# PaddlePaddle/MetaGym

Measured on AMD Instinct MI355X. Metric: env-steps/sec (whole node) at 2^16 parallel envs; 1/2/4/8-GPU scaling, higher is better.
Workload: dtype f32/f64 mixed (reference choreography)

## Files before the change

metagym_amd/csrc/quadrotor.hip:

```cpp
#include <cstdlib>

#include "mg_common.h"
#include "mg_philox.h"

namespace {

#ifndef MG_QUAD_BLOCK
#define MG_QUAD_BLOCK 256
#endif
constexpr int BLOCK = MG_QUAD_BLOCK;
constexpr int WAVES_PER_BLOCK = BLOCK / mg::WAVE;
constexpr int OBS_DIM = 16;

struct QuadK {
    float phi32, phi_over_ra32, inv_jm32, mm32, prec32, ct0_32, ct1_32;
    float quality32, dt32, zoff32, healthy32, fail_range_sq32;
    float lm[4];
    float pc[12];
    float iinv[9];
    float df[9], dm[9];
    float cog[3];
    double prec, half_dt2, half_dt, ct2, quality, inv_quality;
    double min_v, max_v, fail_velocity, fail_w, healthy, xoff, yoff;
    int quality_recip_exact;
    int times, nt, task;
    int auto_reset;
    float init_v_base[3], init_w_base[3];
    double init_v_noisy, init_w_noisy;
    uint64_t seed, env_id_base;
    const int32_t *map;
    int map_h, map_w;
    const float *vtargets;
    int obs_dim;
};

struct Lane {
    float p[3];
    double v[3];
    double w[3];
    float pw[4];
    float R[9];
    double Rd[9];
    float Ri[9];
    double nv, nw;
    float power;
};


__device__ __forceinline__ double dot_row_f32f64(const float *row, const double *x) {
    return fma((double)row[2], x[2], fma((double)row[0], x[0], (double)row[1] * x[1]));
}

__device__ __forceinline__ void mv_f32f64(const float *M, const double *x, double *y) {
#pragma unroll
    for (int r = 0; r < 3; ++r) y[r] = dot_row_f32f64(&M[3 * r], x);
}

__device__ __forceinline__ void mv_f32(const float *M, const float *x, float *y) {
#pragma unroll
    for (int r = 0; r < 2; ++r) y[r] = (M[3 * r] * x[0] + M[3 * r + 1] * x[1]) + M[3 * r + 2] * x[2];
    y[2] = fmaf(M[8], x[2], fmaf(M[6], x[0], M[7] * x[1]));
}

__device__ __forceinline__ void mm_f32(const float *A, const float *B, float *C) {
#pragma unroll
    for (int r = 0; r < 3; ++r)
#pragma unroll
        for (int c = 0; c < 3; ++c)
            C[3 * r + c] = fmaf(A[3 * r + 2], B[6 + c], fmaf(A[3 * r + 1], B[3 + c], A[3 * r] * B[c]));
}

__device__ __forceinline__ void cross_f32(const float *a, const float *b, float *c) {
    float t0 = a[1] * b[2], t1 = a[2] * b[1];
    float t2 = a[2] * b[0], t3 = a[0] * b[2];
    float t4 = a[0] * b[1], t5 = a[1] * b[0];
    c[0] = t0 - t1;
    c[1] = t2 - t3;
    c[2] = t4 - t5;
}

__device__ __forceinline__ double norm3(const double *x) {
    return sqrt(fma(x[2], x[2], fma(x[1], x[1], x[0] * x[0])));
}
__device__ __forceinline__ float sumsq3(const float *x) {
    const float p0 = x[0] * x[0], p1 = x[1] * x[1], p2 = x[2] * x[2];
    return (float)(((double)p0 + (double)p1) + (double)p2);
}

__device__ __forceinline__ void inv3(const float *Af, float *Ainv, double *A) {
#pragma unroll
    for (int i = 0; i < 9; ++i) A[i] = (double)Af[i];
    const double c00 = fma(A[4], A[8], -(A[5] * A[7]));
    const double c01 = fma(A[5], A[6], -(A[3] * A[8]));
    const double c02 = fma(A[3], A[7], -(A[4] * A[6]));
    const double det = fma(A[2], c02, fma(A[1], c01, A[0] * c00));
    const double r = 1.0 / det;
    Ainv[0] = (float)(c00 * r);
    Ainv[3] = (float)(c01 * r);
    Ainv[6] = (float)(c02 * r);
    Ainv[1] = (float)(fma(A[2], A[7], -(A[1] * A[8])) * r);
    Ainv[4] = (float)(fma(A[0], A[8], -(A[2] * A[6])) * r);
    Ainv[7] = (float)(fma(A[1], A[6], -(A[0] * A[7])) * r);
    Ainv[2] = (float)(fma(A[1], A[5], -(A[2] * A[4])) * r);
    Ainv[5] = (float)(fma(A[2], A[3], -(A[0] * A[5])) * r);
    Ainv[8] = (float)(fma(A[0], A[4], -(A[1] * A[3])) * r);
}

template <bool SIMPLE, bool RECIP = false, bool XF = false>
__device__ __forceinline__ void substep(const QuadK &k, Lane &s, const float *eff32, bool want_power) {
    static_assert(!XF || SIMPLE, "the X frame is a SIMPLE configuration");
    float prop_force_z = 0.0f;
    float prop_torque[3] = {0.0f, 0.0f, 0.0f};
    float me[4], pp[4];

    const double bvz = dot_row_f32f64(&s.Ri[6], s.v);
    double xcz[4];
    if (XF) {
        const double c = (double)k.pc[1];
        const double A = s.w[0] * c, B = s.w[1] * c;
        xcz[0] = A - B;
        xcz[1] = A + B;
        xcz[2] = B - A;
        xcz[3] = (-A) - B;
    }

#pragma unroll
    for (int i = 0; i < 4; ++i) {
        const float e32 = eff32[i];
        float phi_w = k.phi32 * s.pw[i];
        me[i] = k.phi_over_ra32 * (e32 - phi_w);
        if (want_power) pp[i] = fabsf(me[i] / k.phi32 * e32);
        float d_prop_w = k.inv_jm32 * (me[i] - k.mm32);
        float w_m = s.pw[i] + k.prec32 * d_prop_w;
        const float *pc = &k.pc[3 * i];
        double cz = XF ? xcz[i] : s.w[0] * (double)pc[1] - s.w[1] * (double)pc[0];
        double v_1 = bvz + cz * (double)(XF ? k.lm[0] : k.lm[i]);
        float t0 = (k.ct0_32 * w_m) * w_m;
        double t1 = (double)(k.ct1_32 * w_m) * v_1;
        double thrust = (double)t0 + t1;
        if (!SIMPLE) {
            double sign = v_1 > 0 ? 1.0 : -1.0;
            thrust = thrust + ((k.ct2 * v_1) * v_1) * sign;
        }
        s.pw[i] = w_m;
        prop_force_z = (float)((double)prop_force_z + thrust);
        const float T = (float)thrust;
        if (XF) {
            const float Tc = T * k.pc[1];
            prop_torque[0] = (i < 2) ? prop_torque[0] + Tc : prop_torque[0] - Tc;
            prop_torque[1] = (i == 1 || i == 2) ? prop_torque[1] + Tc : prop_torque[1] - Tc;
        } else if (SIMPLE) {
            prop_torque[0] += T * pc[1];
            prop_torque[1] += (-T) * pc[0];
        } else {
            float a[3] = {-0.0f, -0.0f, -T};
            float cr[3];
            cross_f32(a, pc, cr);
            prop_torque[0] += cr[0];
            prop_torque[1] += cr[1];
            prop_torque[2] += cr[2];
        }
    }
    prop_torque[2] += ((-me[0] + me[1]) - me[2]) + me[3];

    float DfRi[9];
    double tmp[3], f_drag[3], t_drag[3];
    if (SIMPLE) {
#pragma unroll
        for (int r = 0; r < 3; ++r)
#pragma unroll
            for (int c = 0; c < 3; ++c) DfRi[3 * r + c] = k.df[4 * r] * s.Ri[3 * r + c];
    } else {
        mm_f32(k.df, s.Ri, DfRi);
    }
    mv_f32f64(DfRi, s.v, tmp);
    const double mnv = -s.nv;
#pragma unroll
    for (int c = 0; c < 3; ++c) f_drag[c] = mnv * tmp[c];
    if (SIMPLE) {
#pragma unroll
        for (int c = 0; c < 3; ++c) tmp[c] = (double)k.dm[4 * c] * s.w[c];
    } else {
        mv_f32f64(k.dm, s.w, tmp);
    }
    const double mnw = -s.nw;
#pragma unroll
    for (int c = 0; c < 3; ++c) t_drag[c] = mnw * tmp[c];

    float f_grav[3];
#pragma unroll
    for (int c = 0; c < 3; ++c) f_grav[c] = (s.Ri[3 * c + 2] * -9.8f) * k.quality32;

    double t_all[3], body_acc[3], acc[3];
    float t_grav_neg[3] = {0.0f, 0.0f, 0.0f};
    if (!SIMPLE) {
        float t_grav[3];
        cross_f32(f_grav, k.cog, t_grav);
#pragma unroll
        for (int c = 0; c < 3; ++c) t_grav_neg[c] = -t_grav[c];
    }
#pragma unroll
    for (int c = 0; c < 3; ++c) {
        const float pf = (c == 2) ? prop_force_z : 0.0f;
        double f_all = (double)(pf + f_grav[c]) + f_drag[c];
        t_all[c] = (double)(SIMPLE ? prop_torque[c] : prop_torque[c] + t_grav_neg[c]) + t_drag[c];
        body_acc[c] = (RECIP || k.quality_recip_exact) ? f_all * k.inv_quality : f_all / k.quality;
    }
#pragma unroll
    for (int r = 0; r < 3; ++r)
        acc[r] = fma(s.Rd[3 * r + 2], body_acc[2], fma(s.Rd[3 * r], body_acc[0], s.Rd[3 * r + 1] * body_acc[1]));
#pragma unroll
    for (int c = 0; c < 3; ++c)
        s.p[c] = (float)((double)s.p[c] + (s.v[c] * k.prec + k.half_dt2 * acc[c]));
#pragma unroll
    for (int c = 0; c < 3; ++c) s.v[c] = s.v[c] + k.prec * acc[c];
    if (want_power) s.power = ((pp[0] + pp[1]) + pp[2]) + pp[3];

    double alpha[3], tw[3];
    if (SIMPLE) {
#pragma unroll
        for (int c = 0; c < 3; ++c) alpha[c] = (double)k.iinv[4 * c] * t_all[c];
    } else {
        mv_f32f64(k.iinv, t_all, alpha);
    }
#pragma unroll
    for (int c = 0; c < 3; ++c) tw[c] = s.w[c] + k.half_dt * alpha[c];
    const float s01 = (float)(-tw[2]), s02 = (float)(tw[1]);
    const float s10 = (float)(tw[2]), s12 = (float)(-tw[0]);
    const float s20 = (float)(-tw[1]), s21 = (float)(tw[0]);
#pragma unroll
    for (int r = 0; r < 3; ++r) {
        const float r0 = s.R[3 * r], r1 = s.R[3 * r + 1], r2 = s.R[3 * r + 2];
        const float rs0 = fmaf(r2, s20, fmaf(r1, s10, r0 * 0.0f));
        const float rs1 = fmaf(r2, s21, fmaf(r1, 0.0f, r0 * s01));
        const float rs2 = fmaf(r2, 0.0f, fmaf(r1, s12, r0 * s02));
        s.R[3 * r] = r0 + k.prec32 * rs0;
        s.R[3 * r + 1] = r1 + k.prec32 * rs1;
        s.R[3 * r + 2] = r2 + k.prec32 * rs2;
    }
#pragma unroll
    for (int c = 0; c < 3; ++c) s.w[c] = s.w[c] + k.prec * alpha[c];
    inv3(s.R, s.Ri, s.Rd);
    s.nv = norm3(s.v);
    s.nw = norm3(s.w);
}

__device__ __forceinline__ int failure_code(const QuadK &k, const Lane &s) {
    const int c3 = (s.nw > k.fail_w) ? 3 : 0;
    const int c2 = (s.nv > k.fail_velocity) ? 2 : c3;
    return (sumsq3(s.p) > k.fail_range_sq32) ? 1 : c2;
}

__device__ __forceinline__ void observe(const QuadK &k, const Lane &s, float *obs) {
    double b_v[3];
    float b_pos[3], imu[3];
    const float g[3] = {0.0f, 0.0f, -9.8f};
    mv_f32f64(s.Ri, s.v, b_v);
    mv_f32(s.Ri, s.p, b_pos);
    mv_f32(s.Ri, g, imu);
    float roll = atan2f(s.R[7], s.R[8]);
    float pitch = atan2f(-s.R[6], sqrtf(s.R[7] * s.R[7] + s.R[8] * s.R[8]));
    float yaw = atan2f(s.R[3], s.R[0]);
    obs[0] = (float)b_v[0]; obs[1] = (float)b_v[1]; obs[2] = (float)b_v[2];
    obs[3] = b_pos[0]; obs[4] = b_pos[1]; obs[5] = b_pos[2];
    obs[6] = 0.0f + imu[0]; obs[7] = 0.0f + imu[1]; obs[8] = 0.0f + imu[2];
    obs[9] = (float)s.w[0]; obs[10] = (float)s.w[1]; obs[11] = (float)s.w[2];
    obs[12] = pitch; obs[13] = roll; obs[14] = yaw;
    obs[15] = s.p[2] + k.zoff32;
}

__device__ __forceinline__ void py_slice(long a, long b, long len, long &lo, long &hi) {
    if (a < 0) { a += len; if (a < 0) a = 0; } else if (a > len) a = len;
    if (b < 0) { b += len; if (b < 0) b = 0; } else if (b > len) b = len;
    lo = a; hi = b;
}

__device__ __forceinline__ bool collision(const QuadK &k, const double *op, const double *np_) {
    long mn[3], mx[3];
#pragma unroll
    for (int i = 0; i < 3; ++i) {
        double lo = op[i] < np_[i] ? op[i] : np_[i];
        double hi = op[i] > np_[i] ? op[i] : np_[i];
        mn[i] = (long)floor(lo);
        mx[i] = (long)ceil(hi);
    }
    int any = 0;
    if (k.map != nullptr) {
        long y0, y1, x0, x1;
        py_slice(mn[1], mx[1] + 1, k.map_h, y0, y1);
        py_slice(mn[0], mx[0] + 1, k.map_w, x0, x1);
        for (long y = y0; y < y1; ++y)
            for (long x = x0; x < x1; ++x) any |= (k.map[y * k.map_w + x] != 0);
    }
    return (mn[2] < any) || (mx[2] < any);
}

struct Lane32 {
    float p[3], v[3], w[3], pw[4], R[9], Ri[9];
};

__device__ void substep_f32state(const QuadK &k, Lane32 &s, const float *eff32) {
    float prop_force_z = 0.0f, prop_torque[3] = {0.0f, 0.0f, 0.0f}, me[4];
    const float ct2_32 = (float)k.ct2;
    for (int i = 0; i < 4; ++i) {
        const float e32 = eff32[i];
        float phi_w = k.phi32 * s.pw[i];
        me[i] = k.phi_over_ra32 * (e32 - phi_w);
        float d_prop_w = k.inv_jm32 * (me[i] - k.mm32);
        float w_m = s.pw[i] + k.prec32 * d_prop_w;
        const float *pc = &k.pc[3 * i];
        float bv[3], cr[3];
        mv_f32(s.Ri, s.v, bv);
        cross_f32(s.w, pc, cr);
        float v_1 = bv[2] + cr[2] * k.lm[i];
        float sign = v_1 > 0 ? 1.0f : -1.0f;
        float thrust = ((k.ct0_32 * w_m) * w_m + (k.ct1_32 * w_m) * v_1) + ((ct2_32 * v_1) * v_1) * sign;
        s.pw[i] = w_m;
        prop_force_z = prop_force_z + thrust;
        float a[3] = {-0.0f, -0.0f, -thrust};
        cross_f32(a, pc, cr);
        prop_torque[0] += cr[0]; prop_torque[1] += cr[1]; prop_torque[2] += cr[2];
    }
    prop_torque[2] += ((-me[0] + me[1]) - me[2]) + me[3];
    float DfRi[9], tmp[3], f_drag[3], t_drag[3];
    mm_f32(k.df, s.Ri, DfRi);
    mv_f32(DfRi, s.v, tmp);
    const float nv = -sqrtf(sumsq3(s.v));
    for (int c = 0; c < 3; ++c) f_drag[c] = nv * tmp[c];
    mv_f32(k.dm, s.w, tmp);
    const float nw = -sqrtf(sumsq3(s.w));
    for (int c = 0; c < 3; ++c) t_drag[c] = nw * tmp[c];
    const float g[3] = {0.0f, 0.0f, -9.8f};
    float f_grav[3], t_grav[3], body_acc[3], t_all[3], acc[3];
    mv_f32(s.Ri, g, f_grav);
    for (int c = 0; c < 3; ++c) f_grav[c] = f_grav[c] * k.quality32;
    cross_f32(f_grav, k.cog, t_grav);
    for (int c = 0; c < 3; ++c) {
        const float pf = (c == 2) ? prop_force_z : 0.0f;
        const float f_all = (pf + f_grav[c]) + f_drag[c];
        t_all[c] = (prop_torque[c] + (-t_grav[c])) + t_drag[c];
        body_acc[c] = f_all / k.quality32;
    }
    mv_f32(s.R, body_acc, acc);
    const float half_dt2 = (float)k.half_dt2, half_dt = (float)k.half_dt;
    for (int c = 0; c < 3; ++c) s.p[c] = s.p[c] + (s.v[c] * k.prec32 + half_dt2 * acc[c]);
    for (int c = 0; c < 3; ++c) s.v[c] = s.v[c] + k.prec32 * acc[c];
    float alpha[3], tw[3];
    mv_f32(k.iinv, t_all, alpha);
    for (int c = 0; c < 3; ++c) tw[c] = s.w[c] + half_dt * alpha[c];
    float S[9] = {0.0f, -tw[2], tw[1], tw[2], 0.0f, -tw[0], -tw[1], tw[0], 0.0f};
    float RS[9];
    mm_f32(s.R, S, RS);
    for (int c = 0; c < 9; ++c) s.R[c] = s.R[c] + k.prec32 * RS[c];
    for (int c = 0; c < 3; ++c) s.w[c] = s.w[c] + k.prec32 * alpha[c];
    double Rd[9];
    inv3(s.R, s.Ri, Rd);
}

__global__ void quadrotor_targets_kernel(QuadK k, int nt, const float *actions, float *targets) {
    if (blockIdx.x != 0 || threadIdx.x != 0) return;
    Lane32 s;
    for (int c = 0; c < 3; ++c) { s.p[c] = 0.0f; s.v[c] = 0.0f; s.w[c] = 0.0f; }
    for (int c = 0; c < 4; ++c) s.pw[c] = 0.0f;
    for (int c = 0; c < 9; ++c) { s.R[c] = (c % 4 == 0) ? 1.0f : 0.0f; s.Ri[c] = s.R[c]; }
    for (int t = 0; t < nt; ++t) {
        float eff32[4];
        for (int i = 0; i < 4; ++i) {
            double d = (double)actions[4 * t + i];
            d = d > k.max_v ? k.max_v : (d < k.min_v ? k.min_v : d);
            eff32[i] = (float)d;
        }
        for (int it = 0; it < k.times; ++it) substep_f32state(k, s, eff32);
        targets[3 * t] = s.v[0]; targets[3 * t + 1] = s.v[1]; targets[3 * t + 2] = s.v[2];
    }
}


template <typename T> __device__ __forceinline__ void st_stream(T *p, T v) { __builtin_nontemporal_store(v, p); }
typedef float v4f __attribute__((ext_vector_type(4)));
typedef uint32_t v2u __attribute__((ext_vector_type(2)));
typedef uint32_t v4u __attribute__((ext_vector_type(4)));

constexpr int AUX_NT = 2;
__device__ __forceinline__ __amdgpu_buffer_rsrc_t rsrc_of(const void *base, uint32_t bytes) {
    return __builtin_amdgcn_make_buffer_rsrc(const_cast<void *>(base), (short)0, (int)bytes, 0x00020000);
}
template <typename T> __device__ __forceinline__ T buf_ld(__amdgpu_buffer_rsrc_t r, uint32_t vo, uint32_t so) {
    if constexpr (sizeof(T) == 4) return __builtin_bit_cast(T, __builtin_amdgcn_raw_buffer_load_b32(r, vo, so, 0));
    else if constexpr (sizeof(T) == 8) return __builtin_bit_cast(T, __builtin_amdgcn_raw_buffer_load_b64(r, vo, so, 0));
    else return __builtin_bit_cast(T, __builtin_amdgcn_raw_buffer_load_b128(r, vo, so, 0));
}
template <int AUX, typename T> __device__ __forceinline__ void buf_st(T v, __amdgpu_buffer_rsrc_t r, uint32_t vo, uint32_t so) {
    if constexpr (sizeof(T) == 1) __builtin_amdgcn_raw_buffer_store_b8(__builtin_bit_cast(uint8_t, v), r, vo, so, AUX);
    else if constexpr (sizeof(T) == 4) __builtin_amdgcn_raw_buffer_store_b32(__builtin_bit_cast(uint32_t, v), r, vo, so, AUX);
    else if constexpr (sizeof(T) == 8) __builtin_amdgcn_raw_buffer_store_b64(__builtin_bit_cast(v2u, v), r, vo, so, AUX);
    else __builtin_amdgcn_raw_buffer_store_b128(__builtin_bit_cast(v4u, v), r, vo, so, AUX);
}
template <bool BUF, typename T> __device__ __forceinline__ T ld_soa(const T *a, int comps, int n, int c, int e) {
    if (!BUF) return a[(size_t)c * n + e];
    return buf_ld<T>(rsrc_of(a, (uint32_t)comps * (uint32_t)n * sizeof(T)), (uint32_t)e * sizeof(T),
                     (uint32_t)c * (uint32_t)n * sizeof(T));
}
template <bool BUF, typename T> __device__ __forceinline__ void st_soa(T *a, int comps, int n, int c, int e, T v) {
    if (!BUF) return st_stream(&a[(size_t)c * n + e], v);
    buf_st<AUX_NT>(v, rsrc_of(a, (uint32_t)comps * (uint32_t)n * sizeof(T)), (uint32_t)e * sizeof(T),
                   (uint32_t)c * (uint32_t)n * sizeof(T));
}

template <bool ROT_FIRST = false, bool BUF = false>
__device__ __forceinline__ void load_state(const mg_quadrotor_state &st, int n, int e, Lane &s, int &ct) {
    if (ROT_FIRST) {
#pragma unroll
        for (int c = 0; c < 9; ++c) s.R[c] = ld_soa<BUF>(st.rot, 9, n, c, e);
    }
    if (!ROT_FIRST) {
#pragma unroll
        for (int c = 0; c < 3; ++c) s.p[c] = ld_soa<BUF>(st.pos, 3, n, c, e);
    }
#pragma unroll
    for (int c = 0; c < 3; ++c) s.v[c] = ld_soa<BUF>(st.vel, 3, n, c, e);
#pragma unroll
    for (int c = 0; c < 3; ++c) s.w[c] = ld_soa<BUF>(st.omega, 3, n, c, e);
    if (ROT_FIRST) {
#pragma unroll
        for (int c = 0; c < 3; ++c) s.p[c] = ld_soa<BUF>(st.pos, 3, n, c, e);
    }
#pragma unroll
    for (int c = 0; c < 4; ++c) s.pw[c] = ld_soa<BUF>(st.propw, 4, n, c, e);
    if (!ROT_FIRST) {
#pragma unroll
        for (int c = 0; c < 9; ++c) s.R[c] = ld_soa<BUF>(st.rot, 9, n, c, e);
    }
    ct = ld_soa<BUF>(st.ct, 1, n, 0, e);
}

__device__ __forceinline__ void derive_lane(Lane &s) {
    inv3(s.R, s.Ri, s.Rd);
    s.nv = norm3(s.v);
    s.nw = norm3(s.w);
    s.power = 0.0f;
}

template <bool BUF = false>
__device__ __forceinline__ void load_lane(const mg_quadrotor_state &st, int n, int e, Lane &s, int &ct) {
    load_state<false, BUF>(st, n, e, s, ct);
    derive_lane(s);
}

template <bool BUF = false>
__device__ __forceinline__ void store_lane(const mg_quadrotor_state &st, int n, int e, const Lane &s, int ct) {
#pragma unroll
    for (int c = 0; c < 3; ++c) st_soa<BUF>(st.pos, 3, n, c, e, s.p[c]);
#pragma unroll
    for (int c = 0; c < 3; ++c) st_soa<BUF>(st.vel, 3, n, c, e, s.v[c]);
#pragma unroll
    for (int c = 0; c < 3; ++c) st_soa<BUF>(st.omega, 3, n, c, e, s.w[c]);
#pragma unroll
    for (int c = 0; c < 4; ++c) st_soa<BUF>(st.propw, 4, n, c, e, s.pw[c]);
#pragma unroll
    for (int c = 0; c < 9; ++c) st_soa<BUF>(st.rot, 9, n, c, e, s.R[c]);
    st_soa<BUF>(st.ct, 1, n, 0, e, ct);
}

template <bool BUF = false>
__device__ __forceinline__ void store_obs_wave(float *tile, const float *obs, float *out, int n, int e, int obs_dim) {
    if (!BUF && obs_dim != OBS_DIM) {
        if (e < n)
            for (int c = 0; c < obs_dim; ++c) out[(size_t)e * obs_dim + c] = obs[c];
        return;
    }
    const int lane = threadIdx.x & (mg::WAVE - 1);
    const int wave_base = e - lane;
    const bool full = (wave_base + mg::WAVE) <= n;
    if (full) {
#pragma unroll
        for (int c = 0; c < OBS_DIM; ++c) tile[lane * (OBS_DIM + 1) + c] = obs[c];
        __builtin_amdgcn_wave_barrier();
        float4 *dst = reinterpret_cast<float4 *>(out + (size_t)wave_base * OBS_DIM);
        const __amdgpu_buffer_rsrc_t r = rsrc_of(out, (uint32_t)n * (OBS_DIM * 4));
#pragma unroll
        for (int j = 0; j < 4; ++j) {
            const int q = j * mg::WAVE + lane;
            const int row = q >> 2, col = (q & 3) * 4;
            const float *src = &tile[row * (OBS_DIM + 1) + col];
            const v4f v{src[0], src[1], src[2], src[3]};
            if (BUF) buf_st<AUX_NT>(v, r, (uint32_t)(wave_base * OBS_DIM + 4 * lane) * 4 + j * (mg::WAVE * 16), 0);
            else st_stream(reinterpret_cast<v4f *>(dst + q), v);
        }
        __builtin_amdgcn_wave_barrier();
    } else if (e < n) {
        float4 *dst = reinterpret_cast<float4 *>(out + (size_t)e * OBS_DIM);
        const __amdgpu_buffer_rsrc_t r = rsrc_of(out, (uint32_t)n * (OBS_DIM * 4));
#pragma unroll
        for (int j = 0; j < 4; ++j) {
            const v4f v{obs[4 * j], obs[4 * j + 1], obs[4 * j + 2], obs[4 * j + 3]};
            if (BUF) buf_st<0>(v, r, (uint32_t)e * (OBS_DIM * 4) + j * 16, 0);
            else dst[j] = make_float4(v.x, v.y, v.z, v.w);
        }
    }
}

struct ResetDraw {
    double v[3], w[3], nv, nw;
};

__device__ __forceinline__ ResetDraw reset_draw(const QuadK &k, int e, uint32_t episode) {
    uint32_t r[8];
    const uint64_t gid = k.env_id_base + (uint64_t)e;
#pragma unroll
    for (int b = 0; b < 2; ++b)
        philox4x32_10((uint32_t)gid, (uint32_t)(gid >> 32), episode, (uint32_t)b, (uint32_t)k.seed,
                      (uint32_t)(k.seed >> 32), &r[4 * b]);
    const double inv32 = 1.0 / 4294967296.0;
    ResetDraw d;
#pragma unroll
    for (int c = 0; c < 3; ++c) {
        const double sv = ((r[6] >> c) & 1u) ? 1.0 : -1.0;
        const double sw = ((r[6] >> (3 + c)) & 1u) ? 1.0 : -1.0;
        d.v[c] = (double)k.init_v_base[c] + (k.init_v_noisy * ((double)r[c] * inv32)) * sv;
        d.w[c] = (double)k.init_w_base[c] + (k.init_w_noisy * ((double)r[3 + c] * inv32)) * sw;
    }
    d.nv = norm3(d.v);
    d.nw = norm3(d.w);
    return d;
}

__device__ __forceinline__ void reset_apply(Lane &s, const ResetDraw &d) {
#pragma unroll
    for (int c = 0; c < 3; ++c) {
        s.p[c] = 0.0f;
        s.v[c] = d.v[c];
        s.w[c] = d.w[c];
    }
#pragma unroll
    for (int c = 0; c < 4; ++c) s.pw[c] = 0.0f;
#pragma unroll
    for (int c = 0; c < 9; ++c) {
        s.R[c] = (c % 4 == 0) ? 1.0f : 0.0f;
        s.Ri[c] = s.R[c];
        s.Rd[c] = (double)s.R[c];
    }
    s.nv = d.nv;
    s.nw = d.nw;
    s.power = 0.0f;
}


struct StepIO {
    const float *action;
    float *obs;
    float *reward;
    double *reward64;
    uint8_t *done;
    uint8_t *failed;
};

struct KArgs { QuadK k; mg_quadrotor_state st; StepIO io; int n; int n_steps; };
typedef const __attribute__((address_space(4))) KArgs KArgsC;
__device__ __forceinline__ KArgsC *kernargs_fresh() {
    KArgsC *p = (KArgsC *)__builtin_amdgcn_kernarg_segment_ptr();
    asm volatile("" : "+s"(p));
    return p;
}

enum StepForm { STEP_GENERIC = 0, STEP_STOCK = 1, STEP_STOCK_SHADOW = 2 };
constexpr int STOCK_TIMES = 10;
#ifndef MG_QUAD_SUBSTEP_UNROLL
#define MG_QUAD_SUBSTEP_UNROLL 9
#endif

template <bool SIMPLE, int FORM, bool XF = false, bool BUF = false>
__global__ __launch_bounds__(BLOCK) void quadrotor_step_kernel(QuadK k, mg_quadrotor_state st, StepIO io,
                                                               int n, int n_steps_arg) {
    constexpr bool STOCK = FORM != STEP_GENERIC;
    constexpr bool SHADOW = FORM == STEP_STOCK_SHADOW;
    static_assert(!STOCK || SIMPLE, "the stock forms are SIMPLE");
    static_assert(STOCK || !XF, "XF is an option of the stock forms");
    static_assert(SHADOW || !BUF, "BUF is an option of STEP_STOCK_SHADOW");
    const int n_steps = SHADOW ? 1 : n_steps_arg;
    __shared__ float tiles[WAVES_PER_BLOCK][mg::WAVE * (OBS_DIM + 1)];
    const int e = blockIdx.x * BLOCK + threadIdx.x;
    const bool live = e < n;
    const int el = live ? e : n - 1;
    float *tile = tiles[threadIdx.x / mg::WAVE];

    {
        const uint32_t *ka = (const uint32_t *)__builtin_amdgcn_kernarg_segment_ptr();
        uint32_t touch = 0;
#pragma unroll
        for (int line = 0; line < (int)((sizeof(QuadK) + sizeof(mg_quadrotor_state) + sizeof(StepIO) + 8 + 63) / 64); ++line)
            touch |= ka[line * 16];
        asm volatile("" ::"s"(touch));
    }
    float4 a_next;
    Lane s;
    int ct;
    uint32_t episode = 0;
    ResetDraw rd;
    if (SHADOW) {
        episode = ld_soa<BUF>(st.episode, 1, n, 0, el);
        a_next = ld_soa<BUF>(reinterpret_cast<const float4 *>(io.action), 1, n, 0, el);
        load_state<true, BUF>(st, n, el, s, ct);
        __builtin_amdgcn_sched_barrier(0);
        rd = reset_draw(k, el, episode);
#pragma unroll
        for (int c = 0; c < 3; ++c) asm volatile("" : "+v"(rd.v[c]), "+v"(rd.w[c]));
        asm volatile("" : "+v"(rd.nv), "+v"(rd.nw));
        __builtin_amdgcn_sched_barrier(0);
        derive_lane(s);
        __builtin_amdgcn_sched_barrier(0);
    } else {
        a_next = reinterpret_cast<const float4 *>(io.action)[el];
        __builtin_amdgcn_sched_barrier(0);
        if (STOCK || k.auto_reset) episode = st.episode[el];
        load_lane(st, n, el, s, ct);
    }
    const uint32_t episode_in = episode;
    __builtin_amdgcn_s_waitcnt(0x0F70);

    for (int t = 0; t < n_steps; ++t) {
        const size_t off = (size_t)t * n;
        const float4 a = a_next;
        if (t + 1 < n_steps)
            a_next = reinterpret_cast<const float4 *>(io.action)[off + n + el];
        const float av[4] = {a.x, a.y, a.z, a.w};
        float eff32[4];
#pragma unroll
        for (int i = 0; i < 4; ++i) {
            double d = (double)av[i];
            d = d > k.max_v ? k.max_v : (d < k.min_v ? k.min_v : d);
            eff32[i] = (float)d;
        }
        ct += 1;
        const double old_pos[3] = {(double)s.p[0] + k.xoff, (double)s.p[1] + k.yoff,
                                   (double)(s.p[2] + k.zoff32)};
        int fail = 0;
        if (STOCK) {
#pragma unroll MG_QUAD_SUBSTEP_UNROLL
            for (int it = 0; it < STOCK_TIMES - 1; ++it) {
                substep<SIMPLE, true, XF>(k, s, eff32, false);
                const int code = failure_code(k, s);
                fail = fail ? fail : code;
            }
            substep<SIMPLE, true, XF>(k, s, eff32, true);
            const int code = failure_code(k, s);
            fail = fail ? fail : code;
        } else {
            for (int it = 0; it < k.times; ++it) {
                if (fail == 0) {
                    substep<SIMPLE>(k, s, eff32, it == k.times - 1);
                    fail = failure_code(k, s);
                }
            }
        }
        const KArgsC *kae = kernargs_fresh();
        const QuadK &ke = *(const QuadK *)&kae->k;
        const StepIO &ioe = *(const StepIO *)&kae->io;
        const bool vel_task = ke.task == MG_QUADROTOR_TASK_VELOCITY_CONTROL;
        const int tn_step = ct < ke.nt - 1 ? ct : ke.nt - 1;
        double reward = 0.0;
        int done = 1;
        if (fail == 0 && vel_task) {
            float bt[3];
            mv_f32(s.Ri, &ke.vtargets[3 * (ct - 1)], bt);
            double b_v[3];
            mv_f32f64(s.Ri, s.v, b_v);
            const double diff = (fabs((double)bt[0] - b_v[0]) + fabs((double)bt[1] - b_v[1])) + fabs((double)bt[2] - b_v[2]);
            const float energy = ke.dt32 * s.power;
            const double r = (ke.healthy32 < energy) ? -ke.healthy : -(double)energy;
            reward = r + (-0.001 * diff);
            done = 0;
            if (ct == ke.nt) { done = 1; ct = 0; }
        } else if (fail == 0) {
            const double new_pos[3] = {(double)s.p[0] + ke.xoff, (double)s.p[1] + ke.yoff,
                                       (double)(s.p[2] + ke.zoff32)};
            const bool hit = collision(ke, old_pos, new_pos);
            const float energy = ke.dt32 * s.power;
            double r = (ke.healthy32 < energy) ? -ke.healthy : -(double)energy;
            double task_reward = hit ? 0.0 : ke.healthy;
            if (ke.task == MG_QUADROTOR_TASK_HOVERING_CONTROL) {
                task_reward -= 1.0 * s.nv + 1.0 * s.nw;
                const float z_move = fabsf(0.0f - s.p[2]);
                if (z_move < 0.5f) task_reward += 10;
                else {
                    const float o = 0.5f - z_move;
                    task_reward += (o > -20.0f) ? (double)o : -20.0;
                }
            }
            if (ke.task == MG_QUADROTOR_TASK_HOVERING_CONTROL || ke.healthy32 < energy)
                reward = r + task_reward;
            else
                reward = (double)((float)r + (float)task_reward);
            done = 0;
            if (hit) { done = 1; ct = 0; }
            if (ct == ke.nt) { done = 1; ct = 0; }
        } else {
            ct = 0;
        }
        int tn = tn_step;
        if ((STOCK || ke.auto_reset) && done) {
            if (SHADOW) reset_apply(s, rd);
            else reset_apply(s, reset_draw(ke, el, episode));
            episode += 1;
            tn = ct < ke.nt - 1 ? ct : ke.nt - 1;
        }
        if (t + 1 < n_steps) asm volatile("" : "+v"(a_next.x), "+v"(a_next.y), "+v"(a_next.z), "+v"(a_next.w));
        if (t == n_steps - 1 && live) {
            const mg_quadrotor_state &ste = *(const mg_quadrotor_state *)&kae->st;
            store_lane<BUF>(ste, n, e, s, ct);
            if (episode != episode_in) st_soa<BUF>(ste.episode, 1, n, 0, e, episode);
        }
        __builtin_amdgcn_sched_barrier(0);
        float obs[OBS_DIM + 3];
        observe(ke, s, obs);
        if (vel_task) { obs[16] = ke.vtargets[3 * tn]; obs[17] = ke.vtargets[3 * tn + 1]; obs[18] = ke.vtargets[3 * tn + 2]; }
        store_obs_wave<BUF>(tile, obs, ioe.obs + off * ke.obs_dim, n, e, ke.obs_dim);
        if (live) {
            if (BUF) {
                if (ioe.reward) st_soa<true>(ioe.reward + off, 1, n, 0, e, (float)reward);
                if (ioe.reward64) st_soa<true>(ioe.reward64 + off, 1, n, 0, e, reward);
                st_soa<true>(ioe.done + off, 1, n, 0, e, (uint8_t)done);
                if (ioe.failed) st_soa<true>(ioe.failed + off, 1, n, 0, e, (uint8_t)fail);
            } else {
                if (ioe.reward) st_stream(&ioe.reward[off + e], (float)reward);
                if (ioe.reward64) st_stream(&ioe.reward64[off + e], reward);
                st_stream(&ioe.done[off + e], (uint8_t)done);
                if (ioe.failed) st_stream(&ioe.failed[off + e], (uint8_t)fail);
            }
        }
    }
}

__global__ __launch_bounds__(BLOCK) void quadrotor_reset_kernel(QuadK k, mg_quadrotor_state st,
                                                                const uint8_t *mask, const double *init_vel,
                                                                const double *init_omega, float *obs_out, int n) {
    const int e = blockIdx.x * BLOCK + threadIdx.x;
    if (e >= n) return;
    if (mask != nullptr && mask[e] == 0) return;
    Lane s;
#pragma unroll
    for (int c = 0; c < 3; ++c) {
        s.p[c] = 0.0f;
        s.v[c] = init_vel ? init_vel[(size_t)c * n + e] : 0.0;
        s.w[c] = init_omega ? init_omega[(size_t)c * n + e] : 0.0;
    }
#pragma unroll
    for (int c = 0; c < 4; ++c) s.pw[c] = 0.0f;
#pragma unroll
    for (int c = 0; c < 9; ++c) s.R[c] = (c % 4 == 0) ? 1.0f : 0.0f;
    inv3(s.R, s.Ri, s.Rd);
    s.nv = norm3(s.v);
    s.nw = norm3(s.w);
    s.power = 0.0f;
    const int ct = st.ct[e];
    store_lane(st, n, e, s, ct);
    if (obs_out != nullptr) {
        float obs[OBS_DIM + 3];
        observe(k, s, obs);
        if (k.task == MG_QUADROTOR_TASK_VELOCITY_CONTROL) {
            const int tn = ct < k.nt - 1 ? ct : k.nt - 1;
            obs[16] = k.vtargets[3 * tn]; obs[17] = k.vtargets[3 * tn + 1]; obs[18] = k.vtargets[3 * tn + 2];
        }
        for (int c = 0; c < k.obs_dim; ++c) obs_out[(size_t)e * k.obs_dim + c] = obs[c];
    }
}


void host_inv3_f32(const float *Af, float *Ainv) {
    double A[9];
    for (int i = 0; i < 9; ++i) A[i] = (double)Af[i];
    const double c00 = fma(A[4], A[8], -(A[5] * A[7])), c01 = fma(A[5], A[6], -(A[3] * A[8])),
                 c02 = fma(A[3], A[7], -(A[4] * A[6]));
    const double det = fma(A[2], c02, fma(A[1], c01, A[0] * c00));
    const double r = 1.0 / det;
    Ainv[0] = (float)(c00 * r); Ainv[3] = (float)(c01 * r); Ainv[6] = (float)(c02 * r);
    Ainv[1] = (float)(fma(A[2], A[7], -(A[1] * A[8])) * r);
    Ainv[4] = (float)(fma(A[0], A[8], -(A[2] * A[6])) * r);
    Ainv[7] = (float)(fma(A[1], A[6], -(A[0] * A[7])) * r);
    Ainv[2] = (float)(fma(A[1], A[5], -(A[2] * A[4])) * r);
    Ainv[5] = (float)(fma(A[2], A[3], -(A[0] * A[5])) * r);
    Ainv[8] = (float)(fma(A[0], A[4], -(A[1] * A[3])) * r);
}

int fold_config(const mg_quadrotor_config *c, QuadK *k, bool need_targets = true) {
    if (!(c->precision >= 1e-8) || c->precision > c->dt)
        return mg::set_error(MG_ERR_BAD_CONFIG, "precision %g must be in [1e-8, dt=%g]", c->precision, c->dt);
    if (c->task != MG_QUADROTOR_TASK_NO_COLLISION && c->task != MG_QUADROTOR_TASK_HOVERING_CONTROL &&
        c->task != MG_QUADROTOR_TASK_VELOCITY_CONTROL)
        return mg::set_error(MG_ERR_UNSUPPORTED, "quadrotor task %d is not implemented", c->task);
    if (c->task == MG_QUADROTOR_TASK_VELOCITY_CONTROL && need_targets && c->velocity_targets_d == nullptr)
        return mg::set_error(MG_ERR_NULL_POINTER, "velocity_control needs cfg->velocity_targets_d");
    if (c->map_d != nullptr && (c->map_h <= 0 || c->map_w <= 0))
        return mg::set_error(MG_ERR_BAD_SIZE, "map shape %d x %d", c->map_h, c->map_w);
    k->phi32 = (float)c->phi;
    k->phi_over_ra32 = (float)(c->phi / c->ra);
    k->inv_jm32 = (float)(1.0 / c->jm);
    k->mm32 = (float)c->mm;
    k->prec32 = (float)c->precision;
    k->ct0_32 = (float)c->ct0;
    k->ct1_32 = (float)c->ct1;
    k->quality32 = (float)c->quality;
    k->dt32 = (float)c->dt;
    k->zoff32 = (float)c->z_offset;
    k->healthy32 = (float)c->healthy_reward;
    {
        const float T = (float)c->fail_range;
        float S = T * T;
        while (sqrtf(S) > T) S = nextafterf(S, 0.0f);
        while (sqrtf(nextafterf(S, INFINITY)) <= T) S = nextafterf(S, INFINITY);
        k->fail_range_sq32 = S;
    }
    for (int i = 0; i < 4; ++i) {
        const float *p = &c->prop_coord[3 * i];
        const float p0 = p[0] * p[0], p1 = p[1] * p[1], p2 = p[2] * p[2];
        k->lm[i] = sqrtf((float)(((double)p0 + (double)p1) + (double)p2));
    }
    for (int i = 0; i < 12; ++i) k->pc[i] = c->prop_coord[i];
    host_inv3_f32(c->inertia, k->iinv);
    for (int i = 0; i < 9; ++i) { k->df[i] = c->drag_f[i]; k->dm[i] = c->drag_m[i]; }
    for (int i = 0; i < 3; ++i) k->cog[i] = c->gravity_center[i];
    k->prec = c->precision;
    k->half_dt2 = 0.5 * c->precision * c->precision;
    k->half_dt = 0.5 * c->precision;
    k->ct2 = c->ct2;
    k->quality = c->quality;
    k->inv_quality = 1.0 / c->quality;
    int ex = 0;
    (void)frexp(c->quality, &ex);
    k->quality_recip_exact = (frexp(c->quality, &ex) == 0.5) ? 1 : 0;
    k->min_v = c->min_voltage;
    k->max_v = c->max_voltage;
    k->fail_velocity = c->fail_velocity;
    k->fail_w = c->fail_w;
    k->healthy = c->healthy_reward;
    k->xoff = (double)c->x_offset;
    k->yoff = (double)c->y_offset;
    k->times = (int)(c->dt / c->precision);
    k->nt = c->nt;
    k->task = c->task;
    k->map = c->map_d;
    k->map_h = c->map_h;
    k->map_w = c->map_w;
    k->vtargets = c->velocity_targets_d;
    k->obs_dim = c->task == MG_QUADROTOR_TASK_VELOCITY_CONTROL ? 19 : 16;
    k->auto_reset = 0;
    for (int i = 0; i < 3; ++i) { k->init_v_base[i] = 0.0f; k->init_w_base[i] = 0.0f; }
    k->init_v_noisy = k->init_w_noisy = 0.0;
    k->seed = k->env_id_base = 0;
    return MG_OK;
}

bool config_is_simple(const mg_quadrotor_config *c) {
    for (int r = 0; r < 3; ++r)
        for (int col = 0; col < 3; ++col)
            if (r != col && (c->drag_f[3 * r + col] != 0.0f || c->drag_m[3 * r + col] != 0.0f ||
                             c->inertia[3 * r + col] != 0.0f))
                return false;
    for (int i = 0; i < 3; ++i)
        if (c->gravity_center[i] != 0.0f) return false;
    for (int i = 0; i < 4; ++i)
        if (c->prop_coord[3 * i + 2] != 0.0f) return false;
    return c->ct2 == 0.0;
}

bool config_is_xframe(const mg_quadrotor_config *cfg) {
    const float *pc = cfg->prop_coord;
    const float c = pc[1];
    const float sx[4] = {1.0f, -1.0f, -1.0f, 1.0f}, sy[4] = {1.0f, 1.0f, -1.0f, -1.0f};
    if (!(c > 0.0f && c < INFINITY)) return false;
    for (int i = 0; i < 4; ++i)
        if (pc[3 * i] != sx[i] * c || pc[3 * i + 1] != sy[i] * c || pc[3 * i + 2] != 0.0f) return false;
    return true;
}

int check_state(const mg_quadrotor_state *s) {
    if (!s->pos || !s->vel || !s->omega || !s->propw || !s->rot || !s->ct)
        return mg::set_error(MG_ERR_NULL_POINTER, "mg_quadrotor_state has a NULL array");
    return MG_OK;
}

struct Plan {
    uint32_t magic;
    int32_t n, device, simple;
    int32_t stock;
    int32_t xframe;
    int32_t simds;
    QuadK k;
    mg_quadrotor_state st;
};
constexpr uint32_t PLAN_MAGIC = 0x4d475150u;
static_assert(sizeof(Plan) <= sizeof(mg_quadrotor_plan), "mg_quadrotor_plan is too small for the folded constants");

int make_plan(Plan *p, const mg_quadrotor_config *cfg, const mg_quadrotor_autoreset *ar, int32_t n,
              const mg_quadrotor_state *state) {
    MG_REQUIRE_PTR(cfg);
    MG_REQUIRE_PTR(state);
    if (n <= 0) return mg::set_error(MG_ERR_BAD_SIZE, "n_envs=%d", n);
    if (int rc = check_state(state)) return rc;
    if (int rc = fold_config(cfg, &p->k)) return rc;
    if (ar != nullptr) {
        if (state->episode == nullptr)
            return mg::set_error(MG_ERR_NULL_POINTER, "fused auto-reset needs mg_quadrotor_state.episode");
        QuadK &k = p->k;
        k.auto_reset = 1;
        for (int i = 0; i < 3; ++i) { k.init_v_base[i] = ar->init_velocity[i]; k.init_w_base[i] = ar->init_angular_velocity[i]; }
        k.init_v_noisy = ar->init_velocity_noisy;
        k.init_w_noisy = ar->init_angular_velocity_noisy;
        k.seed = ar->seed;
        k.env_id_base = ar->env_id_base;
    }
    p->magic = PLAN_MAGIC;
    p->n = n;
    p->device = mg::device_of(state->pos);
    p->simple = (config_is_simple(cfg) && cfg->task != MG_QUADROTOR_TASK_VELOCITY_CONTROL) ? 1 : 0;
    const bool force_generic = getenv("MG_QUAD_GENERIC") != nullptr;
    p->stock = (!force_generic && p->simple && p->k.quality_recip_exact && p->k.times == STOCK_TIMES && p->k.auto_reset) ? 1 : 0;
    p->xframe = (p->stock && config_is_xframe(cfg)) ? 1 : 0;
    p->simds = 0;
    int cus = 0;
    if (p->device >= 0 && hipDeviceGetAttribute(&cus, hipDeviceAttributeMultiprocessorCount, p->device) == hipSuccess)
        p->simds = 4 * cus;
    else
        (void)hipGetLastError();
    p->st = *state;
    return MG_OK;
}

int launch_plan(const Plan *p, int32_t n_steps, const float *action, float *obs, float *reward, double *reward64,
                uint8_t *done, uint8_t *failed, void *stream) {
    MG_REQUIRE_PTR(action);
    MG_REQUIRE_PTR(obs);
    MG_REQUIRE_PTR(done);
    if (n_steps <= 0) return mg::set_error(MG_ERR_BAD_SIZE, "n_steps=%d", n_steps);
    mg::DeviceGuard guard(p->device);
    StepIO io{action, obs, reward, reward64, done, failed};
    const int n = p->n, grid = (n + BLOCK - 1) / BLOCK;
    const int waves = (n + mg::WAVE - 1) / mg::WAVE;
    const bool buf = (uint64_t)n * (OBS_DIM * sizeof(float)) < (1ull << 31);
    constexpr int SH = STEP_STOCK_SHADOW;
    decltype(&quadrotor_step_kernel<false, STEP_GENERIC>) kern;
    if (p->stock && n_steps == 1 && waves <= p->simds) {
        if (p->xframe) kern = buf ? quadrotor_step_kernel<true, SH, true, true> : quadrotor_step_kernel<true, SH, true, false>;
        else kern = buf ? quadrotor_step_kernel<true, SH, false, true> : quadrotor_step_kernel<true, SH, false, false>;
    } else if (p->stock) {
        kern = p->xframe ? quadrotor_step_kernel<true, STEP_STOCK, true> : quadrotor_step_kernel<true, STEP_STOCK>;
    } else if (p->simple) {
        kern = quadrotor_step_kernel<true, STEP_GENERIC>;
    } else {
        kern = quadrotor_step_kernel<false, STEP_GENERIC>;
    }
    hipLaunchKernelGGL(kern, dim3(grid), dim3(BLOCK), 0, (hipStream_t)stream, p->k, p->st, io, n, n_steps);
    return mg::check_launch("quadrotor_step_kernel");
}

int launch_steps(const mg_quadrotor_config *cfg, int32_t n, int32_t n_steps, const mg_quadrotor_state *state,
                 const float *action, float *obs, float *reward, double *reward64, uint8_t *done,
                 uint8_t *failed, void *stream, const mg_quadrotor_autoreset *ar = nullptr) {
    MG_REQUIRE_PTR(cfg);
    MG_REQUIRE_PTR(state);
    MG_REQUIRE_PTR(action);
    MG_REQUIRE_PTR(obs);
    MG_REQUIRE_PTR(done);
    Plan p;
    if (int rc = make_plan(&p, cfg, ar, n, state)) return rc;
    return launch_plan(&p, n_steps, action, obs, reward, reward64, done, failed, stream);
}

}

extern "C" int mg_quadrotor_default_config(mg_quadrotor_config *c) {
    MG_REQUIRE_PTR(c);
    *c = mg_quadrotor_config{};
    c->precision = 0.001;
    c->quality = 0.5;
    c->ct0 = 1.538e-5; c->ct1 = -2.5e-4; c->ct2 = 0.0;
    c->mm = 0.010; c->jm = 2.573e-4; c->ra = 0.2010; c->phi = 0.017242179827506;
    c->fail_velocity = 100.0; c->fail_w = 1000.0; c->fail_range = 1000.0;
    c->min_voltage = 0.10; c->max_voltage = 15.0;
    c->dt = 0.01; c->healthy_reward = 1.0; c->z_offset = 5.0;
    c->x_offset = 50; c->y_offset = 50;
    c->nt = 1000;
    c->task = MG_QUADROTOR_TASK_NO_COLLISION;
    c->inertia[0] = 0.0135f; c->inertia[4] = 0.0135f; c->inertia[8] = 0.024f;
    c->drag_m[0] = 0.074f; c->drag_m[4] = 0.074f; c->drag_m[8] = 0.0506f;
    c->drag_f[0] = 0.12f; c->drag_f[4] = 0.12f; c->drag_f[8] = 0.10f;
    const float pc[12] = {0.18f, 0.18f, 0.f, -0.18f, 0.18f, 0.f, -0.18f, -0.18f, 0.f, 0.18f, -0.18f, 0.f};
    for (int i = 0; i < 12; ++i) c->prop_coord[i] = pc[i];
    c->map_d = nullptr; c->map_h = 100; c->map_w = 100;
    return MG_OK;
}

extern "C" int mg_quadrotor_velocity_targets(const mg_quadrotor_config *cfg, int32_t nt, const float *actions_d,
                                             float *targets_d, void *stream) {
    MG_REQUIRE_PTR(cfg);
    MG_REQUIRE_PTR(actions_d);
    MG_REQUIRE_PTR(targets_d);
    if (nt <= 0) return mg::set_error(MG_ERR_BAD_SIZE, "nt=%d", nt);
    QuadK k;
    if (int rc = fold_config(cfg, &k, false)) return rc;
    mg::DeviceGuard guard(mg::device_of(targets_d));
    hipLaunchKernelGGL(quadrotor_targets_kernel, dim3(1), dim3(64), 0, (hipStream_t)stream, k, nt, actions_d, targets_d);
    return mg::check_launch("quadrotor_targets_kernel");
}

extern "C" int mg_quadrotor_reset(const mg_quadrotor_config *cfg, int32_t n, const mg_quadrotor_state *state,
                                  const uint8_t *mask, const double *init_vel, const double *init_omega,
                                  float *obs, void *stream) {
    MG_REQUIRE_PTR(cfg);
    MG_REQUIRE_PTR(state);
    if (n <= 0) return mg::set_error(MG_ERR_BAD_SIZE, "n_envs=%d", n);
    if (int rc = check_state(state)) return rc;
    QuadK k;
    if (int rc = fold_config(cfg, &k)) return rc;
    const int grid = (n + BLOCK - 1) / BLOCK;
    mg::DeviceGuard guard(mg::device_of(state->pos));
    hipLaunchKernelGGL(quadrotor_reset_kernel, dim3(grid), dim3(BLOCK), 0, (hipStream_t)stream, k, *state, mask,
                       init_vel, init_omega, obs, n);
    return mg::check_launch("quadrotor_reset_kernel");
}

extern "C" int mg_quadrotor_step(const mg_quadrotor_config *cfg, int32_t n, const mg_quadrotor_state *state,
                                 const float *action, float *obs, float *reward, double *reward64,
                                 uint8_t *done, uint8_t *failed, void *stream) {
    return launch_steps(cfg, n, 1, state, action, obs, reward, reward64, done, failed, stream);
}

extern "C" int mg_quadrotor_step_autoreset(const mg_quadrotor_config *cfg, int32_t n, int32_t n_steps,
                                           const mg_quadrotor_state *state, const mg_quadrotor_autoreset *ar,
                                           const float *action, float *obs, float *reward, double *reward64,
                                           uint8_t *done, uint8_t *failed, void *stream) {
    MG_REQUIRE_PTR(ar);
    return launch_steps(cfg, n, n_steps, state, action, obs, reward, reward64, done, failed, stream, ar);
}

extern "C" int mg_quadrotor_rollout(const mg_quadrotor_config *cfg, int32_t n, int32_t n_steps,
                                    const mg_quadrotor_state *state, const float *action, float *obs,
                                    float *reward, double *reward64, uint8_t *done, uint8_t *failed,
                                    void *stream) {
    return launch_steps(cfg, n, n_steps, state, action, obs, reward, reward64, done, failed, stream);
}

extern "C" int mg_quadrotor_plan_init(mg_quadrotor_plan *plan, const mg_quadrotor_config *cfg,
                                      const mg_quadrotor_autoreset *ar, int32_t n_envs,
                                      const mg_quadrotor_state *state) {
    MG_REQUIRE_PTR(plan);
    Plan *p = reinterpret_cast<Plan *>(plan);
    p->magic = 0;
    return make_plan(p, cfg, ar, n_envs, state);
}

extern "C" int mg_quadrotor_plan_step(const mg_quadrotor_plan *plan, int32_t n_steps, const float *action, float *obs,
                                      float *reward, double *reward64, uint8_t *done, uint8_t *failed, void *stream) {
    MG_REQUIRE_PTR(plan);
    const Plan *p = reinterpret_cast<const Plan *>(plan);
    if (p->magic != PLAN_MAGIC) return mg::set_error(MG_ERR_BAD_CONFIG, "mg_quadrotor_plan is not initialised");
    return launch_plan(p, n_steps, action, obs, reward, reward64, done, failed, stream);
}
```

Baseline: 4.694 billion.

## Add speculative fast path for quadrotor substeps with wave-level replay fallback

In the shadow stock kernel, each substep's IEEE double division and sqrt are replaced with hardware rcp/rsq plus Newton refinement. This is valid only when the operands lie in a safe exponent range, and ballot masks flag every lane where that does not hold. The change also drops the multiply-by-zero terms in the rotation update, tracks failure codes as wave ballot masks, and after the ten substeps replays the whole step from stored state on the exact path if any lane flagged a range or negative-zero issue. It aims to remove expensive f64 division and sqrt sequences from the hot loop. The cost is extra code, a rare full-wave replay, and reliance on the refinement matching the exactly rounded results.

```diff
diff --git a/metagym_amd/csrc/quadrotor.hip b/metagym_amd/csrc/quadrotor.hip
--- a/metagym_amd/csrc/quadrotor.hip
+++ b/metagym_amd/csrc/quadrotor.hip
@@ -79,22 +79,46 @@
     c[2] = t4 - t5;
 }
 
-__device__ __forceinline__ double norm3(const double *x) {
-    return sqrt(fma(x[2], x[2], fma(x[1], x[1], x[0] * x[0])));
+__device__ __forceinline__ double sumsq3(const double *x) { return fma(x[2], x[2], fma(x[1], x[1], x[0] * x[0])); }
+__device__ __forceinline__ double norm3(const double *x) { return sqrt(sumsq3(x)); }
+
+__device__ __forceinline__ double sqrt_in_range(double x) {
+    const double y = __builtin_amdgcn_rsq(x);
+    double g = x * y, h = y * 0.5;
+    const double r = fma(-h, g, 0.5);
+    g = fma(g, r, g);
+    const double d0 = fma(-g, g, x);
+    h = fma(h, r, h);
+    g = fma(d0, h, g);
+    const double d1 = fma(-g, g, x);
+    return fma(d1, h, g);
+}
+__device__ __forceinline__ bool sq_in_range(double x) {
+    return (uint32_t)__double2hiint(x) - 0x10000000u < 0x6FF00000u;
+}
+__device__ __forceinline__ double rcp_in_range(double d) {
+    double rc = __builtin_amdgcn_rcp(d);
+    rc = fma(rc, fma(-d, rc, 1.0), rc);
+    rc = fma(rc, fma(-d, rc, 1.0), rc);
+    return fma(fma(-d, rc, 1.0), rc, rc);
+}
+__device__ __forceinline__ bool det_in_range(double d) {
+    return ((uint32_t)__double2hiint(d) << 1) - 0x40000000u < 0x80000000u;
 }
 __device__ __forceinline__ float sumsq3(const float *x) {
     const float p0 = x[0] * x[0], p1 = x[1] * x[1], p2 = x[2] * x[2];
     return (float)(((double)p0 + (double)p1) + (double)p2);
 }
 
-__device__ __forceinline__ void inv3(const float *Af, float *Ainv, double *A) {
+template <bool FAST = false>
+__device__ __forceinline__ double inv3(const float *Af, float *Ainv, double *A) {
 #pragma unroll
     for (int i = 0; i < 9; ++i) A[i] = (double)Af[i];
     const double c00 = fma(A[4], A[8], -(A[5] * A[7]));
     const double c01 = fma(A[5], A[6], -(A[3] * A[8]));
     const double c02 = fma(A[3], A[7], -(A[4] * A[6]));
     const double det = fma(A[2], c02, fma(A[1], c01, A[0] * c00));
-    const double r = 1.0 / det;
+    const double r = FAST ? rcp_in_range(det) : 1.0 / det;
     Ainv[0] = (float)(c00 * r);
     Ainv[3] = (float)(c01 * r);
     Ainv[6] = (float)(c02 * r);
@@ -104,10 +128,20 @@
     Ainv[2] = (float)(fma(A[1], A[5], -(A[2] * A[4])) * r);
     Ainv[5] = (float)(fma(A[2], A[3], -(A[0] * A[5])) * r);
     Ainv[8] = (float)(fma(A[0], A[4], -(A[1] * A[3])) * r);
-}
-
-template <bool SIMPLE, bool RECIP = false, bool XF = false>
-__device__ __forceinline__ void substep(const QuadK &k, Lane &s, const float *eff32, bool want_power) {
+    return det;
+}
+
+__device__ __forceinline__ uint64_t fast_inv3_norms(Lane &s) {
+    const double det = inv3<true>(s.R, s.Ri, s.Rd);
+    const double v2 = sumsq3(s.v), w2 = sumsq3(s.w);
+    s.nv = sqrt_in_range(v2);
+    s.nw = sqrt_in_range(w2);
+    return __builtin_amdgcn_ballot_w64(!det_in_range(det)) | __builtin_amdgcn_ballot_w64(!sq_in_range(v2)) |
+           __builtin_amdgcn_ballot_w64(!sq_in_range(w2));
+}
+
+template <bool SIMPLE, bool RECIP = false, bool XF = false, bool FAST = false>
+__device__ __forceinline__ uint64_t substep(const QuadK &k, Lane &s, const float *eff32, bool want_power) {
     static_assert(!XF || SIMPLE, "the X frame is a SIMPLE configuration");
     float prop_force_z = 0.0f;
     float prop_torque[3] = {0.0f, 0.0f, 0.0f};
@@ -231,18 +265,29 @@
 #pragma unroll
     for (int r = 0; r < 3; ++r) {
         const float r0 = s.R[3 * r], r1 = s.R[3 * r + 1], r2 = s.R[3 * r + 2];
-        const float rs0 = fmaf(r2, s20, fmaf(r1, s10, r0 * 0.0f));
-        const float rs1 = fmaf(r2, s21, fmaf(r1, 0.0f, r0 * s01));
-        const float rs2 = fmaf(r2, 0.0f, fmaf(r1, s12, r0 * s02));
+        float rs0, rs1, rs2;
+        if (FAST) {
+            rs0 = fmaf(r2, s20, r1 * s10);
+            rs1 = fmaf(r2, s21, r0 * s01);
+            rs2 = fmaf(r1, s12, r0 * s02);
+        } else {
+            rs0 = fmaf(r2, s20, fmaf(r1, s10, r0 * 0.0f));
+            rs1 = fmaf(r2, s21, fmaf(r1, 0.0f, r0 * s01));
+            rs2 = fmaf(r2, 0.0f, fmaf(r1, s12, r0 * s02));
+        }
         s.R[3 * r] = r0 + k.prec32 * rs0;
         s.R[3 * r + 1] = r1 + k.prec32 * rs1;
         s.R[3 * r + 2] = r2 + k.prec32 * rs2;
     }
 #pragma unroll
     for (int c = 0; c < 3; ++c) s.w[c] = s.w[c] + k.prec * alpha[c];
-    inv3(s.R, s.Ri, s.Rd);
-    s.nv = norm3(s.v);
-    s.nw = norm3(s.w);
+    if (!FAST) {
+        inv3(s.R, s.Ri, s.Rd);
+        s.nv = norm3(s.v);
+        s.nw = norm3(s.w);
+        return 0;
+    }
+    return fast_inv3_norms(s);
 }
 
 __device__ __forceinline__ int failure_code(const QuadK &k, const Lane &s) {
@@ -434,11 +479,23 @@
     ct = ld_soa<BUF>(st.ct, 1, n, 0, e);
 }
 
-__device__ __forceinline__ void derive_lane(Lane &s) {
-    inv3(s.R, s.Ri, s.Rd);
-    s.nv = norm3(s.v);
-    s.nw = norm3(s.w);
+template <bool FAST = false>
+__device__ __forceinline__ uint64_t derive_lane(Lane &s) {
     s.power = 0.0f;
+    if (!FAST) {
+        inv3(s.R, s.Ri, s.Rd);
+        s.nv = norm3(s.v);
+        s.nw = norm3(s.w);
+        return 0;
+    }
+    return fast_inv3_norms(s);
+}
+
+__device__ __forceinline__ bool has_neg_zero(const float *R) {
+    int m = __float_as_int(R[0]);
+#pragma unroll
+    for (int c = 1; c < 9; ++c) m = min(m, __float_as_int(R[c]));
+    return m == INT32_MIN;
 }
 
 template <bool BUF = false>
@@ -568,12 +625,22 @@
 #ifndef MG_QUAD_SUBSTEP_UNROLL
 #define MG_QUAD_SUBSTEP_UNROLL 9
 #endif
+#ifndef MG_QUAD_FASTPATH
+#define MG_QUAD_FASTPATH 1
+#endif
+#ifndef MG_QUAD_COUNT_REPLAYS
+#define MG_QUAD_COUNT_REPLAYS 0
+#endif
+#if MG_QUAD_COUNT_REPLAYS
+__device__ unsigned long long g_quad_replays;
+#endif
 
 template <bool SIMPLE, int FORM, bool XF = false, bool BUF = false>
 __global__ __launch_bounds__(BLOCK) void quadrotor_step_kernel(QuadK k, mg_quadrotor_state st, StepIO io,
                                                                int n, int n_steps_arg) {
     constexpr bool STOCK = FORM != STEP_GENERIC;
     constexpr bool SHADOW = FORM == STEP_STOCK_SHADOW;
+    constexpr bool FAST = SHADOW && MG_QUAD_FASTPATH;
     static_assert(!STOCK || SIMPLE, "the stock forms are SIMPLE");
     static_assert(STOCK || !XF, "XF is an option of the stock forms");
     static_assert(SHADOW || !BUF, "BUF is an option of STEP_STOCK_SHADOW");
@@ -597,6 +664,7 @@
     int ct;
     uint32_t episode = 0;
     ResetDraw rd;
+    uint64_t replay = 0;
     if (SHADOW) {
         episode = ld_soa<BUF>(st.episode, 1, n, 0, el);
         a_next = ld_soa<BUF>(reinterpret_cast<const float4 *>(io.action), 1, n, 0, el);
@@ -607,7 +675,8 @@
         for (int c = 0; c < 3; ++c) asm volatile("" : "+v"(rd.v[c]), "+v"(rd.w[c]));
         asm volatile("" : "+v"(rd.nv), "+v"(rd.nw));
         __builtin_amdgcn_sched_barrier(0);
-        derive_lane(s);
+        replay = derive_lane<FAST>(s);
+        if (FAST) replay |= __builtin_amdgcn_ballot_w64(has_neg_zero(s.R));
         __builtin_amdgcn_sched_barrier(0);
     } else {
         a_next = reinterpret_cast<const float4 *>(io.action)[el];
@@ -635,7 +704,49 @@
         const double old_pos[3] = {(double)s.p[0] + k.xoff, (double)s.p[1] + k.yoff,
                                    (double)(s.p[2] + k.zoff32)};
         int fail = 0;
-        if (STOCK) {
+        if (FAST) {
+            uint64_t f1 = 0, f2 = 0, f3 = 0;
+            auto fast_substep = [&](bool want_power) {
+                const uint64_t out = substep<SIMPLE, true, XF, true>(k, s, eff32, want_power);
+                const uint64_t failed = f1 | f2 | f3;
+                replay |= out & ~failed;
+                const uint64_t m1 = __builtin_amdgcn_ballot_w64(sumsq3(s.p) > k.fail_range_sq32);
+                const uint64_t m2 = __builtin_amdgcn_ballot_w64(s.nv > k.fail_velocity) & ~m1;
+                const uint64_t m3 = __builtin_amdgcn_ballot_w64(s.nw > k.fail_w) & ~(m1 | m2);
+                f1 |= m1 & ~failed;
+                f2 |= m2 & ~failed;
+                f3 |= m3 & ~failed;
+            };
+#pragma unroll MG_QUAD_SUBSTEP_UNROLL
+            for (int it = 0; it < STOCK_TIMES - 1; ++it) fast_substep(false);
+            fast_substep(true);
+#pragma unroll
+            for (int c = 0; c < 3; ++c) asm volatile("" : "+v"(s.p[c]), "+v"(s.v[c]), "+v"(s.w[c]));
+#pragma unroll
+            for (int c = 0; c < 9; ++c) asm volatile("" : "+v"(s.R[c]), "+v"(s.Ri[c]));
+#pragma unroll
+            for (int c = 0; c < 4; ++c) asm volatile("" : "+v"(s.pw[c]));
+            asm volatile("" : "+v"(s.nv), "+v"(s.nw), "+v"(s.power));
+            if (__builtin_expect(replay != 0, 0)) {
+#if MG_QUAD_COUNT_REPLAYS
+                if ((threadIdx.x & (mg::WAVE - 1)) == 0) atomicAdd(&g_quad_replays, 1ull);
+#endif
+                const KArgsC *kar = kernargs_fresh();
+                int ct_loaded;
+                load_state<true, BUF>(*(const mg_quadrotor_state *)&kar->st, n, el, s, ct_loaded);
+                derive_lane(s);
+#pragma unroll 1
+                for (int it = 0; it < STOCK_TIMES; ++it) {
+                    substep<SIMPLE, true, XF>(k, s, eff32, it == STOCK_TIMES - 1);
+                    const int code = failure_code(k, s);
+                    fail = fail ? fail : code;
+                }
+            } else {
+                fail = __builtin_amdgcn_inverse_ballot_w64(f3) ? 3 : 0;
+                fail = __builtin_amdgcn_inverse_ballot_w64(f2) ? 2 : fail;
+                fail = __builtin_amdgcn_inverse_ballot_w64(f1) ? 1 : fail;
+            }
+        } else if (STOCK) {
 #pragma unroll MG_QUAD_SUBSTEP_UNROLL
             for (int it = 0; it < STOCK_TIMES - 1; ++it) {
                 substep<SIMPLE, true, XF>(k, s, eff32, false);
@@ -1040,6 +1151,16 @@
     return launch_steps(cfg, n, n_steps, state, action, obs, reward, reward64, done, failed, stream);
 }
 
+#if MG_QUAD_COUNT_REPLAYS
+extern "C" int mg_quadrotor_debug_replays(unsigned long long *count) {
+    MG_REQUIRE_PTR(count);
+    const unsigned long long zero = 0;
+    if (int rc = mg::check_hip(hipMemcpyFromSymbol(count, HIP_SYMBOL(g_quad_replays), sizeof(zero)), "replay counter"))
+        return rc;
+    return mg::check_hip(hipMemcpyToSymbol(HIP_SYMBOL(g_quad_replays), &zero, sizeof(zero)), "replay counter");
+}
+#endif
+
 extern "C" int mg_quadrotor_plan_init(mg_quadrotor_plan *plan, const mg_quadrotor_config *cfg,
                                       const mg_quadrotor_autoreset *ar, int32_t n_envs,
                                       const mg_quadrotor_state *state) {
```

After: 4.820 billion, median of 6. 1.03x the previous value.
